# craftsangjae/instance-segmentation-road-project

Hardware: AMD Instinct MI355X
Metric: images/sec at 1024x1024 (MaskLab inference hot path, full forward) (higher is better)
Workload: dtype f32; 1 GPU; resnext50_full_b8_1024; per_gpu_batch=8, global_batch=8, height=1024, width=1024, parallelism=dp1, hipgraph=False, inputs=resident in HBM, weights=random init (cls logits x8 so NMS / mask head run at full load)

## Files before the change

instance-segmentation-road-project_amd/csrc/conv_wino.hip:

```cpp
#include "common.h"

namespace {

constexpr int WMAXP = ML_CONV_MAX_PROBLEMS;
constexpr int WT = 64;
constexpr int WN = 32;
constexpr int WK = 8;
constexpr int PT_LD = 132;
constexpr int WB_LD = 516;
constexpr int WCHUNK = WK * WN * 16;

struct WProblem {
    ml_conv2d_desc d;
    int TH, TW, T;
    int MB, NB, nchunks;
};

struct WArgs {
    int n;
    int start[WMAXP + 1];
    WProblem p[WMAXP];
};

__device__ __forceinline__ void bt_d_b(const float d[16], float v[16]) {
    float t[16];
#pragma unroll
    for (int j = 0; j < 4; ++j) {
        t[0 * 4 + j] = d[0 * 4 + j] - d[2 * 4 + j];
        t[1 * 4 + j] = d[1 * 4 + j] + d[2 * 4 + j];
        t[2 * 4 + j] = d[2 * 4 + j] - d[1 * 4 + j];
        t[3 * 4 + j] = d[1 * 4 + j] - d[3 * 4 + j];
    }
#pragma unroll
    for (int i = 0; i < 4; ++i) {
        v[i * 4 + 0] = t[i * 4 + 0] - t[i * 4 + 2];
        v[i * 4 + 1] = t[i * 4 + 1] + t[i * 4 + 2];
        v[i * 4 + 2] = t[i * 4 + 2] - t[i * 4 + 1];
        v[i * 4 + 3] = t[i * 4 + 1] - t[i * 4 + 3];
    }
}

__global__ void __launch_bounds__(256, 2) conv_wino_kernel(const WArgs args) {
    __shared__ __attribute__((aligned(16))) float lds_p[WT * PT_LD];
    __shared__ __attribute__((aligned(16))) float lds_w[WK * WB_LD];
    __shared__ double lds_gn[4][4];

    int pi = 0;
    while (pi + 1 < args.n && (int)blockIdx.x >= args.start[pi + 1]) ++pi;
    const WProblem &P = args.p[pi];
    const ml_conv2d_desc &p = P.d;
    const int b = (int)blockIdx.x - args.start[pi];
    const int g = b / (8 * P.NB), rr = b - g * 8 * P.NB;
    const int nt = rr >> 3;
    const int mt = g * 8 + (rr & 7);
    if (mt >= P.MB) return;
    if (p.live) {
        const int lv = max(1, *p.live), tpi0 = P.TH * P.TW;
        const int b0 = mt * WT / tpi0, b1 = min(mt * WT + WT, P.T) - 1;
        bool any = false;
        for (int bi = b0; bi <= b1 / tpi0 && !any; ++bi) any = bi % p.live_period < lv;
        if (!any) return;
    }

    const int tid = threadIdx.x, lane = tid & 63, wave = tid >> 6;
    const int r = lane & 15, kq = lane >> 4;
    const int tpi = P.TH * P.TW;

    int pix[8];
#pragma unroll
    for (int i = 0; i < 8; ++i) {
        const int idx = tid + 256 * i;
        const int tile = idx >> 5, px = (idx >> 1) & 15;
        const int gt = mt * WT + tile;
        pix[i] = -1;
        if (gt < P.T) {
            const int bi = gt / tpi, rem = gt - bi * tpi;
            const int ty = rem / P.TW, tx = rem - ty * P.TW;
            const int y = 2 * ty - 1 + (px >> 2), x = 2 * tx - 1 + (px & 3);
            if (y >= 0 && y < p.H && x >= 0 && x < p.W) pix[i] = (bi * p.H + y) * p.W + x;
        }
    }
    const size_t cstride = (size_t)p.in_cstride;
    const float *in = p.in + p.in_coff + ((tid & 1) << 2);
    const float *wsrc = p.wgt + (size_t)nt * P.nchunks * WCHUNK + tid * 4;

    f32x4 rp[8], rw[4];
    auto load_chunk = [&](int c) {
#pragma unroll
        for (int i = 0; i < 8; ++i) {
            rp[i] = f32x4{0.f, 0.f, 0.f, 0.f};
            if (pix[i] >= 0) rp[i] = *reinterpret_cast<const f32x4 *>(in + (size_t)pix[i] * cstride + c * WK);
        }
#pragma unroll
        for (int i = 0; i < 4; ++i) rw[i] = *reinterpret_cast<const f32x4 *>(wsrc + (size_t)c * WCHUNK + i * 1024);
    };

    f32x4 acc[2][16];
#pragma unroll
    for (int t = 0; t < 2; ++t)
#pragma unroll
        for (int q = 0; q < 16; ++q) acc[t][q] = f32x4{0.f, 0.f, 0.f, 0.f};

    load_chunk(0);
    for (int c = 0; c < P.nchunks; ++c) {
        __syncthreads();
#pragma unroll
        for (int i = 0; i < 8; ++i) {
            const int idx = tid + 256 * i;
            *reinterpret_cast<f32x4 *>(lds_p + (idx >> 5) * PT_LD + (idx & 31) * 4) = rp[i];
        }
#pragma unroll
        for (int i = 0; i < 4; ++i) {
            const int idx = tid + 256 * i;
            *reinterpret_cast<f32x4 *>(lds_w + (idx >> 7) * WB_LD + (idx & 127) * 4) = rw[i];
        }
        __syncthreads();
        if (c + 1 < P.nchunks) load_chunk(c + 1);
#pragma unroll
        for (int s = 0; s < 2; ++s) {
            const int ch = 4 * s + kq;
            const float *pa = lds_p + (wave * 16 + r) * PT_LD + ch;
            float d[16], v[16];
#pragma unroll
            for (int px = 0; px < 16; ++px) d[px] = pa[px * WK];
            bt_d_b(d, v);
#pragma unroll
            for (int t = 0; t < 2; ++t) {
                const float *pb = lds_w + ch * WB_LD + (16 * t + r) * 16;
#pragma unroll
                for (int pq = 0; pq < 4; ++pq) {
                    const f32x4 bq = *reinterpret_cast<const f32x4 *>(pb + 4 * pq);
#pragma unroll
                    for (int e = 0; e < 4; ++e)
                        acc[t][4 * pq + e] = __builtin_amdgcn_mfma_f32_16x16x4f32(v[4 * pq + e], bq[e], acc[t][4 * pq + e], 0, 0, 0);
                }
            }
        }
    }

    const bool gn = p.gn_partials != nullptr;
    double gs[2] = {0.0, 0.0}, gq[2] = {0.0, 0.0};
    long long f0 = 0;
    if (gn) {
        const int gt0 = mt * WT;
        const int bi = gt0 / tpi, rem = gt0 - bi * tpi, ty = rem / P.TW, tx = rem - ty * P.TW;
        f0 = ((long long)(bi * p.Ho + 2 * ty) * p.Wo + 2 * tx) >> 7;
    }
    const float lo = 0.f, hi = (p.act == ML_ACT_RELU6) ? 6.f : 3.402823466e38f;
    const bool clampv = p.act == ML_ACT_RELU || p.act == ML_ACT_RELU6;
#pragma unroll
    for (int i = 0; i < 4; ++i) {
        const int gt = mt * WT + wave * 16 + kq * 4 + i;
        if (gt >= P.T) continue;
        const int bi = gt / tpi, rem = gt - bi * tpi;
        const int ty = rem / P.TW, tx = rem - ty * P.TW;
        const int oy = 2 * ty, ox = 2 * tx;
        const bool y1 = oy + 1 < p.Ho, x1 = ox + 1 < p.Wo;
        const size_t img = p.out_bstride ? (size_t)bi * (size_t)p.out_bstride : (size_t)bi * p.Ho * p.Wo * p.out_cstride;
        const size_t pix0 = (size_t)oy * p.Wo + ox;
#pragma unroll
        for (int t = 0; t < 2; ++t) {
            const int n = nt * WN + 16 * t + r;
            if (n >= p.cout) continue;
            float m[16];
#pragma unroll
            for (int q = 0; q < 16; ++q) m[q] = acc[t][q][i];
            float u[8];
#pragma unroll
            for (int j = 0; j < 4; ++j) {
                u[j] = m[0 * 4 + j] + m[1 * 4 + j] + m[2 * 4 + j];
                u[4 + j] = m[1 * 4 + j] - m[2 * 4 + j] - m[3 * 4 + j];
            }
            float yv[4];
#pragma unroll
            for (int a = 0; a < 2; ++a) {
                yv[2 * a] = u[4 * a + 0] + u[4 * a + 1] + u[4 * a + 2];
                yv[2 * a + 1] = u[4 * a + 1] - u[4 * a + 2] - u[4 * a + 3];
            }
            const float bv = p.bias ? p.bias[n] : 0.f;
            float *o = p.out + img + p.out_coff + n;
#pragma unroll
            for (int a = 0; a < 2; ++a)
#pragma unroll
                for (int c2 = 0; c2 < 2; ++c2) {
                    if ((a && !y1) || (c2 && !x1)) continue;
                    float val = yv[2 * a + c2] + bv;
                    if (clampv) val = __builtin_amdgcn_fmed3f(val, lo, hi);
                    else if (p.act != ML_ACT_NONE) val = ml_apply_act(val, p.act);
                    o[(pix0 + (size_t)a * p.Wo + c2) * p.out_cstride] = val;
                    if (gn) {
                        const long long m_flat = ((long long)(bi * p.Ho + oy + a) * p.Wo + ox + c2);
                        const int f = (m_flat >> 7) != f0;
                        gs[f] += (double)val;
                        gq[f] += (double)val * (double)val;
                    }
                }
        }
    }
    if (gn) {
#pragma unroll
        for (int o = 32; o > 0; o >>= 1) {
#pragma unroll
            for (int f = 0; f < 2; ++f) {
                gs[f] += __shfl_down(gs[f], o, 64);
                gq[f] += __shfl_down(gq[f], o, 64);
            }
        }
        if (lane == 0) {
            lds_gn[wave][0] = gs[0]; lds_gn[wave][1] = gq[0];
            lds_gn[wave][2] = gs[1]; lds_gn[wave][3] = gq[1];
        }
        __syncthreads();
        if (tid < 2) {
            const int gt1 = mt * WT + WT - 1;
            const int bi = gt1 / tpi, rem = gt1 - bi * tpi, ty = rem / P.TW, tx = rem - ty * P.TW;
            const long long f1 = ((long long)(bi * p.Ho + 2 * ty + 1) * p.Wo + 2 * tx + 1) >> 7;
            const long long ft = tid ? f1 : f0;
            double s = 0.0, q = 0.0;
            for (int w = 0; w < 4; ++w) { s += lds_gn[w][2 * tid]; q += lds_gn[w][2 * tid + 1]; }
            p.gn_partials[2 * (ft * 4 + nt)] = s;
            p.gn_partials[2 * (ft * 4 + nt) + 1] = q;
        }
    }
}

}

extern "C" int ml_conv2d_wino_eligible(const ml_conv2d_desc *d) {
    if (!d) return 0;
    return d->math == ML_MATH_F32 && d->KH == 3 && d->KW == 3 && d->stride == 1 && d->dil == 1 && d->pad_t == 1 &&
           d->pad_l == 1 && d->Ho == d->H && d->Wo == d->W && d->cpp_shift == 30 && d->group_cin_step == 0 &&
           !d->shuffle2x2 && !d->residual && !d->out_f16 && d->span % 32 == 0 && d->span_pad == d->span &&
           d->cout <= 128 && d->n_pad == 128;
}

int ml_conv2d_wino_gn_ok(const ml_conv2d_desc &d) {
    if (d.Ho % 2 || d.Wo % 2 || d.cout != 128 || d.out_bstride || d.act == ML_ACT_SIGMOID) return 0;
    const long long TH = d.Ho / 2, TW = d.Wo / 2;
    return (64 % TW == 0 || TW % 64 == 0) && (TH * TW) % 64 == 0;
}

int ml_conv2d_wino_launch(const ml_conv2d_desc *descs, int n, hipStream_t s) {
    ML_REQUIRE(n >= 1 && n <= WMAXP, "conv2d (winograd): need 1..%d problems", WMAXP);
    WArgs args;
    args.n = n;
    long long start = 0;
    for (int i = 0; i < n; ++i) {
        const ml_conv2d_desc &d = descs[i];
        ML_REQUIRE(ml_conv2d_wino_eligible(&d),
                   "conv2d: tile = 6 (Winograd F(2x2,3x3)) needs ML_MATH_F32, a 3x3 stride-1 undilated 'same' conv, no "
                   "groups / shuffle / residual / half output, span %% 32 == 0 and n_pad == 128");
        ML_REQUIRE(((d.in_cstride | d.in_coff) & 3) == 0 && ml_aligned16(d.in) && ml_aligned16(d.wgt),
                   "conv2d (winograd): 16-byte aligned input channels and weights");
        if (d.gn_partials)
            ML_REQUIRE(ml_conv2d_wino_gn_ok(d) && !d.live, "conv2d (winograd): gn_partials needs even Ho / Wo, Wo / 2 dividing or a "
                                                "multiple of 64, (Ho / 2) (Wo / 2) %% 64 == 0, cout = 128, dense output");
        WProblem &P = args.p[i];
        P.d = d;
        P.TH = (d.Ho + 1) / 2;
        P.TW = (d.Wo + 1) / 2;
        const long long T = (long long)d.B * P.TH * P.TW;
        ML_REQUIRE(T < (1ll << 30), "conv2d (winograd): too many tiles");
        P.T = (int)T;
        P.MB = (int)((T + WT - 1) / WT);
        P.NB = d.n_pad / WN;
        P.nchunks = d.span_pad / WK;
        args.start[i] = (int)start;
        start += (long long)(P.MB + 7) / 8 * 8 * P.NB;
        ML_REQUIRE(start < (1ll << 31), "conv2d (winograd): grid too large");
    }
    args.start[n] = (int)start;
    long long tiles128 = 0;
    bool any_gn = false;
    for (int i = 0; i < n; ++i) {
        tiles128 += ((long long)descs[i].B * descs[i].Ho * descs[i].Wo + 127) / 128 * (descs[i].n_pad / 128);
        any_gn = any_gn || descs[i].gn_partials != nullptr;
    }
    ML_REQUIRE(!any_gn || tiles128 >= ml_conv2d_gn_min_launch_tiles(),
               "conv2d (winograd): gn_partials needs a launch of ml_conv2d_gn_min_launch_tiles() tiles of 128 x 128");
    hipLaunchKernelGGL(conv_wino_kernel, dim3((unsigned)start), dim3(256), 0, s, args);
    ML_CHECK_LAUNCH("conv2d (winograd)");
    return ML_OK;
}
```

Measured before the change: 399.9 images/sec.

## Double-buffer Winograd conv with direct global-to-LDS loads and wider N tile

Restructures the Winograd 3x3 conv kernel to use 512-thread blocks covering 64 output channels (two wave halves split N), with double-buffered LDS staging filled by global_load_lds_dwordx4 instead of register round-trips. XOR swizzles replace the padded LDS layouts to avoid bank conflicts, and each thread now transforms two channels per chunk. The intent is to overlap global loads with MFMA work, drop the VGPR staging and extra barrier per chunk, and halve the redundant input-tile loads across N blocks. It relies on inline asm that manipulates M0, uses a device-side zero buffer for padding pixels, and drops occupancy to one block per CU.

New measurement: 401.5 images/sec (median of 6 runs). No clear change (+0.4%).

```diff
diff --git a/instance-segmentation-road-project_amd/csrc/conv_wino.hip b/instance-segmentation-road-project_amd/csrc/conv_wino.hip
--- a/instance-segmentation-road-project_amd/csrc/conv_wino.hip
+++ b/instance-segmentation-road-project_amd/csrc/conv_wino.hip
@@ -4,11 +4,11 @@
 
 constexpr int WMAXP = ML_CONV_MAX_PROBLEMS;
 constexpr int WT = 64;
-constexpr int WN = 32;
+constexpr int WN = 64;
 constexpr int WK = 8;
-constexpr int PT_LD = 132;
-constexpr int WB_LD = 516;
-constexpr int WCHUNK = WK * WN * 16;
+constexpr int WCHUNK = WK * 32 * 16;
+constexpr int ST_P = WT * 128;
+constexpr int ST = ST_P + 2 * WCHUNK;
 
 struct WProblem {
     ml_conv2d_desc d;
@@ -22,6 +22,14 @@
     WProblem p[WMAXP];
 };
 
+__device__ __attribute__((aligned(16))) float wino_zero[4];
+
+__device__ __forceinline__ void glds16(const float *src, unsigned lds_base) {
+    unsigned keep;
+    asm volatile("s_mov_b32 %0, m0\n\ts_mov_b32 m0, %2\n\ts_nop 0\n\tglobal_load_lds_dwordx4 %1, off\n\ts_mov_b32 m0, %0"
+                 : "=&s"(keep) : "v"(src), "s"(lds_base) : "memory");
+}
+
 __device__ __forceinline__ void bt_d_b(const float d[16], float v[16]) {
     float t[16];
 #pragma unroll
@@ -40,10 +48,8 @@
     }
 }
 
-__global__ void __launch_bounds__(256, 2) conv_wino_kernel(const WArgs args) {
-    __shared__ __attribute__((aligned(16))) float lds_p[WT * PT_LD];
-    __shared__ __attribute__((aligned(16))) float lds_w[WK * WB_LD];
-    __shared__ double lds_gn[4][4];
+__global__ void __launch_bounds__(512, 1) conv_wino_kernel(const WArgs args) {
+    __shared__ __attribute__((aligned(16))) float lds[2 * ST];
 
     int pi = 0;
     while (pi + 1 < args.n && (int)blockIdx.x >= args.start[pi + 1]) ++pi;
@@ -51,7 +57,7 @@
     const ml_conv2d_desc &p = P.d;
     const int b = (int)blockIdx.x - args.start[pi];
     const int g = b / (8 * P.NB), rr = b - g * 8 * P.NB;
-    const int nt = rr >> 3;
+    const int nb = rr >> 3;
     const int mt = g * 8 + (rr & 7);
     if (mt >= P.MB) return;
     if (p.live) {
@@ -62,16 +68,19 @@
         if (!any) return;
     }
 
-    const int tid = threadIdx.x, lane = tid & 63, wave = tid >> 6;
+    const int tid = threadIdx.x, lane = tid & 63;
+    const int wave = __builtin_amdgcn_readfirstlane(tid >> 6);
     const int r = lane & 15, kq = lane >> 4;
+    const int tg = wave & 3, nh = wave >> 2;
     const int tpi = P.TH * P.TW;
-
-    int pix[8];
-#pragma unroll
-    for (int i = 0; i < 8; ++i) {
-        const int idx = tid + 256 * i;
-        const int tile = idx >> 5, px = (idx >> 1) & 15;
-        const int gt = mt * WT + tile;
+    const unsigned lds0 = (unsigned)(uintptr_t)(__attribute__((address_space(3))) float *)lds;
+
+    int pix[4];
+    const float *in = p.in + p.in_coff;
+#pragma unroll
+    for (int i = 0; i < 4; ++i) {
+        const int tile = 2 * (4 * wave + i) + (lane >> 5), jj = (lane & 31) ^ (tile & 15);
+        const int px = jj >> 1, gt = mt * WT + tile;
         pix[i] = -1;
         if (gt < P.T) {
             const int bi = gt / tpi, rem = gt - bi * tpi;
@@ -80,19 +89,25 @@
             if (y >= 0 && y < p.H && x >= 0 && x < p.W) pix[i] = (bi * p.H + y) * p.W + x;
         }
     }
+    const float *wsrc[4];
+#pragma unroll
+    for (int i = 0; i < 4; ++i) {
+        const int q = 4 * wave + i, h = q >> 4, j = (q & 15) * 64 + lane;
+        const int k = j >> 7, n = (j >> 2) & 31, pq = (j & 3) ^ ((n >> 2) & 3);
+        wsrc[i] = p.wgt + (size_t)(2 * nb + h) * P.nchunks * WCHUNK + k * 512 + n * 16 + pq * 4;
+    }
     const size_t cstride = (size_t)p.in_cstride;
-    const float *in = p.in + p.in_coff + ((tid & 1) << 2);
-    const float *wsrc = p.wgt + (size_t)nt * P.nchunks * WCHUNK + tid * 4;
-
-    f32x4 rp[8], rw[4];
-    auto load_chunk = [&](int c) {
-#pragma unroll
-        for (int i = 0; i < 8; ++i) {
-            rp[i] = f32x4{0.f, 0.f, 0.f, 0.f};
-            if (pix[i] >= 0) rp[i] = *reinterpret_cast<const f32x4 *>(in + (size_t)pix[i] * cstride + c * WK);
-        }
-#pragma unroll
-        for (int i = 0; i < 4; ++i) rw[i] = *reinterpret_cast<const f32x4 *>(wsrc + (size_t)c * WCHUNK + i * 1024);
+    const int half4 = ((lane ^ (lane >> 5)) & 1) * 4;
+    auto stage = [&](int c, int s) {
+        const unsigned base = lds0 + (unsigned)(s * ST) * 4u;
+#pragma unroll
+        for (int i = 0; i < 4; ++i) {
+            const float *src = wino_zero;
+            if (pix[i] >= 0) src = in + (size_t)pix[i] * cstride + c * WK + half4;
+            glds16(src, base + (unsigned)(4 * wave + i) * 1024u);
+        }
+#pragma unroll
+        for (int i = 0; i < 4; ++i) glds16(wsrc[i] + (size_t)c * WCHUNK, base + (unsigned)(ST_P + (4 * wave + i) * 256) * 4u);
     };
 
     f32x4 acc[2][16];
@@ -101,41 +116,41 @@
 #pragma unroll
         for (int q = 0; q < 16; ++q) acc[t][q] = f32x4{0.f, 0.f, 0.f, 0.f};
 
-    load_chunk(0);
+    stage(0, 0);
+    asm volatile("s_waitcnt vmcnt(0)" ::: "memory");
+    __syncthreads();
     for (int c = 0; c < P.nchunks; ++c) {
-        __syncthreads();
-#pragma unroll
-        for (int i = 0; i < 8; ++i) {
-            const int idx = tid + 256 * i;
-            *reinterpret_cast<f32x4 *>(lds_p + (idx >> 5) * PT_LD + (idx & 31) * 4) = rp[i];
-        }
-#pragma unroll
-        for (int i = 0; i < 4; ++i) {
-            const int idx = tid + 256 * i;
-            *reinterpret_cast<f32x4 *>(lds_w + (idx >> 7) * WB_LD + (idx & 127) * 4) = rw[i];
-        }
-        __syncthreads();
-        if (c + 1 < P.nchunks) load_chunk(c + 1);
+        const int cur = c & 1;
+        if (c + 1 < P.nchunks) stage(c + 1, cur ^ 1);
+        const float *pa = lds + cur * ST + (tg * 16 + r) * 128 + 2 * (kq & 1);
+        float d0[16], d1[16], v0[16], v1[16];
+#pragma unroll
+        for (int px = 0; px < 16; ++px) {
+            const float2 e = *reinterpret_cast<const float2 *>(pa + (((2 * px + (kq >> 1)) ^ r) << 2));
+            d0[px] = e.x;
+            d1[px] = e.y;
+        }
+        bt_d_b(d0, v0);
+        bt_d_b(d1, v1);
+        const float *pw = lds + cur * ST + ST_P + nh * WCHUNK + r * 16;
+        const int sw = (r >> 2) & 3;
 #pragma unroll
         for (int s = 0; s < 2; ++s) {
-            const int ch = 4 * s + kq;
-            const float *pa = lds_p + (wave * 16 + r) * PT_LD + ch;
-            float d[16], v[16];
-#pragma unroll
-            for (int px = 0; px < 16; ++px) d[px] = pa[px * WK];
-            bt_d_b(d, v);
+            const float *v = s ? v1 : v0;
 #pragma unroll
             for (int t = 0; t < 2; ++t) {
-                const float *pb = lds_w + ch * WB_LD + (16 * t + r) * 16;
+                const float *pb = pw + (2 * kq + s) * 512 + t * 256;
 #pragma unroll
                 for (int pq = 0; pq < 4; ++pq) {
-                    const f32x4 bq = *reinterpret_cast<const f32x4 *>(pb + 4 * pq);
+                    const f32x4 bq = *reinterpret_cast<const f32x4 *>(pb + ((pq ^ sw) << 2));
 #pragma unroll
                     for (int e = 0; e < 4; ++e)
                         acc[t][4 * pq + e] = __builtin_amdgcn_mfma_f32_16x16x4f32(v[4 * pq + e], bq[e], acc[t][4 * pq + e], 0, 0, 0);
                 }
             }
         }
+        asm volatile("s_waitcnt vmcnt(0)" ::: "memory");
+        __syncthreads();
     }
 
     const bool gn = p.gn_partials != nullptr;
@@ -150,7 +165,7 @@
     const bool clampv = p.act == ML_ACT_RELU || p.act == ML_ACT_RELU6;
 #pragma unroll
     for (int i = 0; i < 4; ++i) {
-        const int gt = mt * WT + wave * 16 + kq * 4 + i;
+        const int gt = mt * WT + tg * 16 + kq * 4 + i;
         if (gt >= P.T) continue;
         const int bi = gt / tpi, rem = gt - bi * tpi;
         const int ty = rem / P.TW, tx = rem - ty * P.TW;
@@ -160,7 +175,7 @@
         const size_t pix0 = (size_t)oy * p.Wo + ox;
 #pragma unroll
         for (int t = 0; t < 2; ++t) {
-            const int n = nt * WN + 16 * t + r;
+            const int n = nb * WN + nh * 32 + 16 * t + r;
             if (n >= p.cout) continue;
             float m[16];
 #pragma unroll
@@ -206,20 +221,22 @@
                 gq[f] += __shfl_down(gq[f], o, 64);
             }
         }
+        double *lds_gn = reinterpret_cast<double *>(lds);
         if (lane == 0) {
-            lds_gn[wave][0] = gs[0]; lds_gn[wave][1] = gq[0];
-            lds_gn[wave][2] = gs[1]; lds_gn[wave][3] = gq[1];
+            lds_gn[4 * wave + 0] = gs[0]; lds_gn[4 * wave + 1] = gq[0];
+            lds_gn[4 * wave + 2] = gs[1]; lds_gn[4 * wave + 3] = gq[1];
         }
         __syncthreads();
-        if (tid < 2) {
+        if (tid < 4) {
             const int gt1 = mt * WT + WT - 1;
             const int bi = gt1 / tpi, rem = gt1 - bi * tpi, ty = rem / P.TW, tx = rem - ty * P.TW;
             const long long f1 = ((long long)(bi * p.Ho + 2 * ty + 1) * p.Wo + 2 * tx + 1) >> 7;
-            const long long ft = tid ? f1 : f0;
+            const int f = tid & 1, h = tid >> 1, slot = 2 * nb + h;
+            const long long ft = f ? f1 : f0;
             double s = 0.0, q = 0.0;
-            for (int w = 0; w < 4; ++w) { s += lds_gn[w][2 * tid]; q += lds_gn[w][2 * tid + 1]; }
-            p.gn_partials[2 * (ft * 4 + nt)] = s;
-            p.gn_partials[2 * (ft * 4 + nt) + 1] = q;
+            for (int w = 4 * h; w < 4 * h + 4; ++w) { s += lds_gn[4 * w + 2 * f]; q += lds_gn[4 * w + 2 * f + 1]; }
+            p.gn_partials[2 * (ft * 4 + slot)] = s;
+            p.gn_partials[2 * (ft * 4 + slot) + 1] = q;
         }
     }
 }
@@ -278,7 +295,7 @@
     }
     ML_REQUIRE(!any_gn || tiles128 >= ml_conv2d_gn_min_launch_tiles(),
                "conv2d (winograd): gn_partials needs a launch of ml_conv2d_gn_min_launch_tiles() tiles of 128 x 128");
-    hipLaunchKernelGGL(conv_wino_kernel, dim3((unsigned)start), dim3(256), 0, s, args);
+    hipLaunchKernelGGL(conv_wino_kernel, dim3((unsigned)start), dim3(512), 0, s, args);
     ML_CHECK_LAUNCH("conv2d (winograd)");
     return ML_OK;
 }
```
